# nickirk/pymes

Hardware: AMD Instinct MI355X
Metric: ccsd_iteration_time (lower is better)
Workload: dtype f64

## Files before the change

### pymes_amd/csrc/kernels.hip

```cpp
#include <hip/hip_runtime.h>
#include <type_traits>

#include <algorithm>
#include <atomic>
#include <chrono>
#include <cmath>
#include <cstdio>
#include <cstdlib>
#include <cstring>
#include <mutex>
#include <stdexcept>
#include <string>
#include <vector>

#include "../../include/pymes_amd.h"
#include "device_api.h"
#include "diis_small.h"
#include "device_util.h"
#include "launch.h"

namespace {

constexpr int kThreads = 256;
constexpr int BK = 16;

struct GemmK {
    const double* A;
    const double* B;
    double* C;
    const double* Cin;
    long a_ld, b_ld, ldc;
    int M, N, K;
    int Mc, Nc;
    double alpha, beta;
    int tiles_m, tiles_n;
    int nsplit, kchunk;
    long tile_begin;
    long nb2;
    long a_b1, a_b2, b_b1, b_b2, c_b1, c_b2;
    double* ws;
    long whole = 0, tail = 0;
    int mixed = 0;
    int fat = 0;
};
__host__ __device__ inline long glds_fat_slot(int fat) { return (long)((fat & 1) ? 144 : 128) * ((fat & 2) ? 144 : 128); }

__device__ __forceinline__ long xcd_remap(long b, long nblk) {
    const long q = nblk >> 3, r = nblk & 7;
    const long xcd = b & 7, pos = b >> 3;
    return (xcd < r ? xcd * (q + 1) : r * (q + 1) + (xcd - r) * q) + pos;
}

__device__ __forceinline__ void gemm_tile_rc(const GemmK& g, const long gt, int& tm, int& tn) {
    const int tiles = g.tiles_m * g.tiles_n;
    const int t = (int)(gt - (gt / tiles) * tiles);
    int rows = g.tiles_m, cols = g.tiles_n;
    if (g.fat) {
        rows -= g.fat & 1;
        cols -= (g.fat >> 1) & 1;
        int e = t - rows * cols;
        if (e >= 0) {
            if (g.fat & 1) {
                if (e < cols) { tm = rows; tn = e; return; }
                e -= cols;
            }
            tm = e;
            tn = cols;
            return;
        }
    }
    const int group_sz = 8 * cols;
    const int grp = t / group_sz;
    const int gm = min(rows - grp * 8, 8);
    const int tin = t - grp * group_sz;
    tm = grp * 8 + tin % gm;
    tn = tin / gm;
}

template <int BM, int BN, bool AKC, bool BKC, int VEC, bool STREAM = false>
__device__ __forceinline__ void dgemm_body(const GemmK& g, const long bid) {
    extern __shared__ __attribute__((aligned(16))) double smem[];
    constexpr int WM = BM / 2, WN = BN / 2;
    constexpr int FM = WM / 16, FN = WN / 16;
    constexpr int A_PITCH = AKC ? (BK + 2) : (BM + 16);
    constexpr int A_ROWS = AKC ? BM : BK;
    constexpr int A_TILE = A_PITCH * A_ROWS;
    constexpr int B_PITCH = BKC ? (BK + 2) : (BN + 16);
    constexpr int B_ROWS = BKC ? BN : BK;
    constexpr int B_TILE = B_PITCH * B_ROWS;
    constexpr int LA = BM * BK / (kThreads * VEC);
    constexpr int LB = BN * BK / (kThreads * VEC);
    constexpr int A_CH = (AKC ? BK : BM) / VEC;
    constexpr int B_CH = (BKC ? BK : BN) / VEC;
    constexpr int A_RSTEP = kThreads / A_CH;
    constexpr int B_RSTEP = kThreads / B_CH;

    double* As = smem;
    double* Bs = smem + (STREAM ? 1 : 2) * A_TILE;

    const int tid = threadIdx.x;
    const int lane = tid & 63, wave = tid >> 6;
    const int wm = wave >> 1, wn = wave & 1;
    const int l15 = lane & 15, l4 = lane >> 4;

    const int tiles = g.tiles_m * g.tiles_n;
    const long lt = bid / g.nsplit;
    const int ks = (int)(bid - lt * g.nsplit);
    const long gt = g.tile_begin + lt;
    const long z = gt / tiles;
    const int t = (int)(gt - z * tiles);
    constexpr int GROUP = 8;
    const int group_sz = GROUP * g.tiles_n;
    const int grp = t / group_sz;
    const int first_m = grp * GROUP;
    const int gm = min(g.tiles_m - first_m, GROUP);
    const int tin = t - grp * group_sz;
    const int tm = first_m + tin % gm;
    const int tn = tin / gm;
    const long z1 = z / g.nb2, z2 = z - z1 * g.nb2;

    const double* __restrict__ A = g.A + z1 * g.a_b1 + z2 * g.a_b2;
    const double* __restrict__ B = g.B + z1 * g.b_b1 + z2 * g.b_b2;
    const int m0 = tm * BM, n0 = tn * BN;
    const int kbeg = ks * g.kchunk;
    const int kend = min(g.K, kbeg + g.kchunk);
    const int nkt = (kend - kbeg + BK - 1) / BK;

    const int a_r = tid / A_CH, a_c = (tid % A_CH) * VEC;
    const int b_r = tid / B_CH, b_c = (tid % B_CH) * VEC;
    const double* pa[LA];
    const double* pb[LB];
#pragma unroll
    for (int i = 0; i < LA; ++i) {
        const int r = a_r + i * A_RSTEP;
        if (AKC) pa[i] = A + (long)min(m0 + r, g.M - 1) * g.a_ld + (kbeg + a_c);
        else pa[i] = A + (long)(kbeg + r) * g.a_ld + min(m0 + a_c, g.Mc - VEC);
    }
#pragma unroll
    for (int i = 0; i < LB; ++i) {
        const int r = b_r + i * B_RSTEP;
        if (BKC) pb[i] = B + (long)min(n0 + r, g.N - 1) * g.b_ld + (kbeg + b_c);
        else pb[i] = B + (long)(kbeg + r) * g.b_ld + min(n0 + b_c, g.Nc - VEC);
    }
    const long a_step = AKC ? (long)BK : (long)BK * g.a_ld;
    const long b_step = BKC ? (long)BK : (long)BK * g.b_ld;

    double ra[LA * VEC], rb[LB * VEC];

    auto load_full = [&]() {
#pragma unroll
        for (int i = 0; i < LA; ++i) {
            if constexpr (VEC == 2) {
                const v2d v = *reinterpret_cast<const v2d*>(pa[i]);
                ra[2 * i] = v[0];
// ... 1770 lines not shown
        if (c < nv && d < nv && c >= d) {
            const double x1 = sA[y][tx], x2 = sB[tx][y];
            Vp[row * npp + (long)c * (c + 1) / 2 + d] = x1 + x2;
            if (c > d) Vm[row * npm + (long)c * (c - 1) / 2 + d] = (a > b) ? x1 - x2 : 0.0;
        }
    }
}

constexpr int kFacK = 16;
__global__ void __launch_bounds__(256) ladder_pack_V_factors_kernel(const double* __restrict__ B, double* __restrict__ Vp,
                                                                    double* __restrict__ Vm, int naux, int n, int no, long rp0,
                                                                    long ntp, long npp, long npm) {
    __shared__ double sAc[kFacK][33], sBc[kFacK][33], sAd[kFacK][33], sBd[kFacK][33];
    const long bid = blockIdx.x;
    const long row = bid / ntp;
    const long tp = bid - row * ntp;
    int a, b, tc, td;
    unrank_pair(rp0 + row, a, b);
    unrank_pair(tp, tc, td);
    const int nv = n - no, c0 = tc * 32, d0 = td * 32;
    const long nn = (long)n * n;
    const double* __restrict__ Ba = B + (long)(no + a) * n + no;
    const double* __restrict__ Bb = B + (long)(no + b) * n + no;
    const int t = threadIdx.x, lane = t & 63, w = t >> 6;
    const int wc = (w >> 1) * 16, wd = (w & 1) * 16, l15 = lane & 15, l4 = lane >> 4;
    const int lx = t & 31, lk = t >> 5;
    v4d X = {0.0, 0.0, 0.0, 0.0}, Y = {0.0, 0.0, 0.0, 0.0};
    for (int q0 = 0; q0 < naux; q0 += kFacK) {
#pragma unroll
        for (int h = 0; h < 2; ++h) {
            const int k = lk + 8 * h, q = q0 + k;
            const long qo = (long)q * nn;
            const bool cok = q < naux && c0 + lx < nv, dok = q < naux && d0 + lx < nv;
            sAc[k][lx] = cok ? Ba[qo + c0 + lx] : 0.0;
            sBc[k][lx] = cok ? Bb[qo + c0 + lx] : 0.0;
            sAd[k][lx] = dok ? Ba[qo + d0 + lx] : 0.0;
            sBd[k][lx] = dok ? Bb[qo + d0 + lx] : 0.0;
        }
        __syncthreads();
#pragma unroll
        for (int kk = 0; kk < kFacK; kk += 4) {
            const int k = kk + l4;
            X = __builtin_amdgcn_mfma_f64_16x16x4f64(sAc[k][wc + l15], sBd[k][wd + l15], X, 0, 0, 0);
            Y = __builtin_amdgcn_mfma_f64_16x16x4f64(sBc[k][wc + l15], sAd[k][wd + l15], Y, 0, 0, 0);
        }
        __syncthreads();
    }
    const int d = d0 + wd + l15;
#pragma unroll
    for (int i = 0; i < 4; ++i) {
        const int c = c0 + wc + l4 + 4 * i;
        if (c < nv && d < nv && c >= d) {
            Vp[row * npp + (long)c * (c + 1) / 2 + d] = X[i] + Y[i];
            if (c > d) Vm[row * npm + (long)c * (c - 1) / 2 + d] = (a > b) ? X[i] - Y[i] : 0.0;
        }
    }
}

constexpr int kDirT = 64, kDirK = 8, kDirP = 80;
__global__ void __launch_bounds__(256, 4) direct_rows_fused_kernel(const double* __restrict__ Bvv, double* __restrict__ Vp,
                                                                double* __restrict__ Vm, int nv, int xp, long apitch, int nstage,
                                                                long rp0, long ntp, long npp, long npm) {
    __shared__ __attribute__((aligned(16))) double sm[2][4][kDirK][kDirP];
    const long bid = blockIdx.x;
    const long row = bid / ntp;
    const long tp = bid - row * ntp;
    int a, b, tc, td;
    unrank_pair(rp0 + row, a, b);
    unrank_pair(tp, tc, td);
    const int c0 = tc * kDirT, d0 = td * kDirT;
    const int t = threadIdx.x, lane = t & 63, w = t >> 6;
    const int wc = (w >> 1) * 32, wd = (w & 1) * 32, l15 = lane & 15, l4 = lane >> 4;
    const bool work = c0 + wc < nv && d0 + wd < nv && c0 + wc + 31 >= d0 + wd;
    const int sk = t >> 5, sx = (t & 31) * 2;
    const double* __restrict__ gA = Bvv + a * apitch + (long)sk * xp + sx;
    const double* __restrict__ gB = Bvv + b * apitch + (long)sk * xp + sx;
    const long step = (long)kDirK * xp;
    v2d r0, r1, r2, r3;
    auto fetch = [&](long o) {
        r0 = *reinterpret_cast<const v2d*>(gA + o + c0);
        r1 = *reinterpret_cast<const v2d*>(gB + o + d0);
        r2 = *reinterpret_cast<const v2d*>(gB + o + c0);
        r3 = *reinterpret_cast<const v2d*>(gA + o + d0);
    };
    auto stash = [&](int buf) {
        *reinterpret_cast<v2d*>(&sm[buf][0][sk][sx]) = r0;
        *reinterpret_cast<v2d*>(&sm[buf][1][sk][sx]) = r1;
        *reinterpret_cast<v2d*>(&sm[buf][2][sk][sx]) = r2;
        *reinterpret_cast<v2d*>(&sm[buf][3][sk][sx]) = r3;
    };
    fetch(0);
    stash(0);
    __syncthreads();
    v4d X[2][2], Y[2][2];
#pragma unroll
    for (int i = 0; i < 2; ++i)
#pragma unroll
        for (int j = 0; j < 2; ++j) X[i][j] = Y[i][j] = v4d{0.0, 0.0, 0.0, 0.0};
    for (int st = 0; st < nstage; ++st) {
        const int buf = st & 1;
        const bool more = st + 1 < nstage;
        if (more) fetch((long)(st + 1) * step);
        if (work) {
#pragma unroll
            for (int kk = 0; kk < kDirK; kk += 4) {
                const int k = kk + l4;
                double xa[2], xb[2], ya[2], yb[2];
#pragma unroll
                for (int i = 0; i < 2; ++i) {
                    xa[i] = sm[buf][0][k][wc + 16 * i + l15];
                    xb[i] = sm[buf][1][k][wd + 16 * i + l15];
                    ya[i] = sm[buf][2][k][wc + 16 * i + l15];
                    yb[i] = sm[buf][3][k][wd + 16 * i + l15];
                }
#pragma unroll
                for (int i = 0; i < 2; ++i)
#pragma unroll
                    for (int j = 0; j < 2; ++j) {
                        X[i][j] = __builtin_amdgcn_mfma_f64_16x16x4f64(xa[i], xb[j], X[i][j], 0, 0, 0);
                        Y[i][j] = __builtin_amdgcn_mfma_f64_16x16x4f64(ya[i], yb[j], Y[i][j], 0, 0, 0);
                    }
            }
        }
        if (more) stash(buf ^ 1);
        __syncthreads();
    }
    if (!work) return;
    double* __restrict__ vp = Vp + row * npp;
    double* __restrict__ vm = Vm + row * npm;
#pragma unroll
    for (int i = 0; i < 2; ++i)
#pragma unroll
        for (int j = 0; j < 2; ++j) {
            const int d = d0 + wd + 16 * j + l15;
#pragma unroll
            for (int e = 0; e < 4; ++e) {
                const int c = c0 + wc + 16 * i + l4 + 4 * e;
                if (c < nv && d < nv && c >= d) {
                    vp[(long)c * (c + 1) / 2 + d] = X[i][j][e] + Y[i][j][e];
                    if (c > d) vm[(long)c * (c - 1) / 2 + d] = (a > b) ? X[i][j][e] - Y[i][j][e] : 0.0;
                }
            }
        }
}

__global__ void ladder_dress_tfrag_kernel(const double* __restrict__ t1, double* __restrict__ tf, int no, int nv, int nk, long total) {
    const long e = blockIdx.x * (long)blockDim.x + threadIdx.x;
    if (e >= total) return;
    const int L = (int)(e & 63), kk = (int)((e >> 6) % nk), tile = (int)((e >> 6) / nk);
    const int a = 16 * tile + (L & 15), k = 4 * kk + (L >> 4);
    tf[e] = (a < nv && k < no) ? -t1[(long)a * no + k] : 0.0;
}

template <int NK>
__global__ void __launch_bounds__(64) ladder_dress_kernel(const double* __restrict__ V, const double* __restrict__ Pk,
                                                          const double* __restrict__ tf, double* __restrict__ W, int no,
                                                          int nv, long ld, long row0, long row1, double sgn, long ntp) {
    constexpr int TP = 16 * 16 + 16;
    __shared__ double turn[16 * TP];
    const int lane = threadIdx.x, g = lane >> 4, c = lane & 15;
    const long idx = blockIdx.x >> 3;
    const long cdb = (blockIdx.x & 7) + 8 * (idx / ntp), tp = idx % ntp;
    if (cdb * 16 >= ld) return;
    int ta_, tb_;
    unrank_pair(tp, ta_, tb_);
    const int a0 = ta_ * 16, b0 = tb_ * 16;
    const long tri0 = (long)a0 * (a0 + 1) / 2;
    if (tri0 + (long)15 * a0 + 120 + b0 + 15 < row0 || tri0 + b0 >= row1) return;
    double ta[NK], tb[NK];
#pragma unroll
    for (int kk = 0; kk < NK; ++kk) {
        ta[kk] = tf[((long)ta_ * NK + kk) * 64 + lane];
        tb[kk] = tf[((long)tb_ * NK + kk) * 64 + lane];
    }
    typedef unsigned v2u __attribute__((ext_vector_type(2)));
    constexpr unsigned kOff = 0x80000000u;
    const long col = cdb * 16 + c;
    const unsigned lo = (unsigned)(8 * ((long)g * ld + col));
    const unsigned lo_last = (unsigned)(8 * ((long)(min(4 * (NK - 1) + g, no - 1) - 4 * (NK - 1)) * ld + col));
    const unsigned ldb = (unsigned)(8 * ld);
    const __amdgpu_buffer_rsrc_t rPa = __builtin_amdgcn_make_buffer_rsrc(const_cast<double*>(Pk + (long)a0 * no * ld), 0, kOff, 0x00020000);
    const __amdgpu_buffer_rsrc_t rPb = __builtin_amdgcn_make_buffer_rsrc(const_cast<double*>(Pk + (long)b0 * no * ld), 0, kOff, 0x00020000);
    const __amdgpu_buffer_rsrc_t rV = __builtin_amdgcn_make_buffer_rsrc(const_cast<double*>(V + (tri0 - row0) * ld), 0, kOff, 0x00020000);
    const __amdgpu_buffer_rsrc_t rW = __builtin_amdgcn_make_buffer_rsrc(W + (tri0 - row0) * ld, 0, kOff, 0x00020000);
    unsigned vo[4];
#pragma unroll
    for (int r = 0; r < 4; ++r) {
        const long a = a0 + g + 4 * r;
        vo[r] = a < nv ? (unsigned)(8 * ((a * (a + 1) / 2 - tri0) * ld + col)) : kOff;
    }
    auto row_off = [&](int r, int x) {
        const int a = a0 + g + 4 * r;
        const long row = (long)a * (a + 1) / 2 + x;
        return (x <= a && row >= row0 && row < row1) ? vo[r] : kOff;
    };
    constexpr int PA = 1, NBP = 2 * (PA + 1), VA = 3, NBV = 2 * (VA + 1);
    double pf[NBP][NK], vin[NBV][4];
    auto fetch_p = [&](int n) {
        const int x0 = n < 16 ? a0 : b0, i = n < 16 ? n : n - 16;
        const unsigned so = (unsigned)(min(x0 + i, nv - 1) - x0) * (unsigned)no * ldb;
        const __amdgpu_buffer_rsrc_t rs = n < 16 ? rPa : rPb;
#pragma unroll
        for (int kk = 0; kk < NK - 1; ++kk)
            pf[n % NBP][kk] = __builtin_bit_cast(double, __builtin_amdgcn_raw_buffer_load_b64(rs, lo, so + 4u * kk * ldb, 0));
        pf[n % NBP][NK - 1] = __builtin_bit_cast(double, __builtin_amdgcn_raw_buffer_load_b64(rs, lo_last, so + 4u * (NK - 1) * ldb, 0));
    };
    auto fetch_v = [&](int n) {
        const int x = b0 + n - 16;
#pragma unroll
        for (int r = 0; r < 4; ++r)
            vin[n % NBV][r] = __builtin_bit_cast(double, __builtin_amdgcn_raw_buffer_load_b64(rV, row_off(r, x), (unsigned)x * ldb, 2));
    };
#pragma unroll
    for (int n = 0; n < 2 * PA; ++n) fetch_p(n);
#pragma unroll
    for (int p = 0; p < 8; ++p) {
        const int n0 = 2 * p, n1 = n0 + 1;
        fetch_p(n0 + 2 * PA);
        fetch_p(n1 + 2 * PA);
        if (n0 + 2 * VA >= 16) { fetch_v(n0 + 2 * VA); fetch_v(n1 + 2 * VA); }
        v4d acc0 = {0.0, 0.0, 0.0, 0.0}, acc1 = {0.0, 0.0, 0.0, 0.0};
#pragma unroll
        for (int kk = 0; kk < NK; ++kk) {
            acc0 = __builtin_amdgcn_mfma_f64_16x16x4f64(tb[kk], pf[n0 % NBP][kk], acc0, 0, 0, 0);
            acc1 = __builtin_amdgcn_mfma_f64_16x16x4f64(tb[kk], pf[n1 % NBP][kk], acc1, 0, 0, 0);
        }
#pragma unroll
        for (int rb = 0; rb < 4; ++rb) {
            turn[n0 * TP + (g + 4 * rb) * 16 + c] = acc0[rb];
            turn[n1 * TP + (g + 4 * rb) * 16 + c] = acc1[rb];
        }
    }
    __builtin_amdgcn_fence(__ATOMIC_SEQ_CST, "wavefront");
    __builtin_amdgcn_wave_barrier();
    const double s2 = sgn > 0.0 ? -1.0 : 1.0;
#pragma unroll
    for (int p = 0; p < 8; ++p) {
        const int b = 2 * p, n0 = 16 + b, n1 = n0 + 1;
        if (n0 + 2 * PA < 32) { fetch_p(n0 + 2 * PA); fetch_p(n1 + 2 * PA); }
        if (n0 + 2 * VA < 32) { fetch_v(n0 + 2 * VA); fetch_v(n1 + 2 * VA); }
        v4d acc0, acc1;
#pragma unroll
        for (int r = 0; r < 4; ++r) {
            acc0[r] = fma(s2, turn[(g + 4 * r) * TP + b * 16 + c], vin[n0 % NBV][r]);
            acc1[r] = fma(s2, turn[(g + 4 * r) * TP + (b + 1) * 16 + c], vin[n1 % NBV][r]);
        }
#pragma unroll
        for (int kk = 0; kk < NK; ++kk) {
            acc0 = __builtin_amdgcn_mfma_f64_16x16x4f64(ta[kk], pf[n0 % NBP][kk], acc0, 0, 0, 0);
            acc1 = __builtin_amdgcn_mfma_f64_16x16x4f64(ta[kk], pf[n1 % NBP][kk], acc1, 0, 0, 0);
        }
#pragma unroll
        for (int h = 0; h < 2; ++h) {
            const int bb = b0 + b + h;
#pragma unroll
            for (int r = 0; r < 4; ++r) {
                const double val = (sgn > 0.0 && a0 + g + 4 * r == bb) ? 0.0 : (double)(h ? acc1[r] : acc0[r]);
                __builtin_amdgcn_raw_buffer_store_b64(__builtin_bit_cast(v2u, val), rW, row_off(r, bb), (unsigned)bb * ldb, 2);
            }
        }
    }
}

struct PackTK {
    const double* T; const double* t1; double* Sp; double* Am;
    long ldp, ldm, rp0;
    int no, nv, flags;
};
__device__ __forceinline__ void ladder_pack_T_body(const PackTK& k, const unsigned vb) {
    const double* __restrict__ T = k.T;
    const double* __restrict__ t1 = k.t1;
    double* __restrict__ Sp = k.Sp;
    double* __restrict__ Am = k.Am;
    const int no = k.no, nv = k.nv, flags = k.flags;
    const long ldp = k.ldp, ldm = k.ldm;
    const long row = k.rp0 + vb;
    int c, d;
    unrank_pair(row, c, d);
    const bool row_half = flags & dev::PACK_ROW_HALF, prow = flags & dev::PACK_AM_PROWS,
               col_half = flags & dev::PACK_COL_HALF, pcol = flags & dev::PACK_AM_PCOLS;
    const long o2 = (long)no * no;
    const double* __restrict__ T1 = T ? T + ((long)c * nv + d) * o2 : nullptr;
    const double* __restrict__ T2 = T ? T + ((long)d * nv + c) * o2 : nullptr;
    const double fr = (c == d && row_half) ? 0.25 : 0.5;
    const long mrow = prow ? row : (long)c * (c - 1) / 2 + d;
    const bool has_m = prow || c > d;
    if (threadIdx.x == 0) {
        const long opp = (long)no * (no + 1) / 2, mcols = pcol ? opp : opp - no;
        if (ldp > opp) Sp[row * ldp + opp] = 0.0;
        if (has_m && ldm > mcols) Am[mrow * ldm + mcols] = 0.0;
    }
    for (int e = threadIdx.x; e < o2; e += blockDim.x) {
        const int i = e / no, j = e - i * no;
        if (i < j) continue;
        double x1 = 0.0, x2 = 0.0;
        if (T) { x1 = T1[e]; x2 = T2[e]; }
        if (t1) {
            x1 += t1[(long)c * no + i] * t1[(long)d * no + j];
            x2 += t1[(long)d * no + i] * t1[(long)c * no + j];
        }
        Sp[row * ldp + (long)i * (i + 1) / 2 + j] = ((i == j && col_half) ? 0.5 * fr : fr) * (x1 + x2);
        if (has_m && (pcol || i > j)) {
            const long mcol = pcol ? (long)i * (i + 1) / 2 + j : (long)i * (i - 1) / 2 + j;
            Am[mrow * ldm + mcol] = (c > d && i > j) ? 0.5 * (x1 - x2) : 0.0;
        }
    }
}
__global__ void ladder_pack_T_kernel(const PackTK k) { ladder_pack_T_body(k, blockIdx.x); }

struct UnpackK {
    const double* L; double* R;
    double beta;
    long total;
    int no, nv;
};
__device__ __forceinline__ void ladder_unpack_body(const UnpackK& k, const unsigned vb, const unsigned vgrid) {
    const double* __restrict__ L = k.L;
    double* __restrict__ R = k.R;
    const double beta = k.beta;
    const int no = k.no, nv = k.nv;
    const long total = k.total;
    const long opp = (long)no * (no + 1) / 2, ld = (long)no * no;
    for (long idx = vb * (long)blockDim.x + threadIdx.x; idx < total; idx += (long)vgrid * blockDim.x) {
        long r = idx;
        const int j = (int)(r % no); r /= no;
        const int i = (int)(r % no); r /= no;
        const int b = (int)(r % nv);
        const int a = (int)(r / nv);
        const int ah = max(a, b), al = min(a, b), ih = max(i, j), il = min(i, j);
        const double* __restrict__ row = L + ((long)ah * (ah + 1) / 2 + al) * ld;
        double v = row[(long)ih * (ih + 1) / 2 + il];
        if (a != b && i != j) {
            const double x = row[opp + (long)ih * (ih - 1) / 2 + il];
            v += ((a > b) == (i > j)) ? x : -x;
        }
        R[idx] = (beta != 0.0) ? beta * R[idx] + v : v;
    }
}
__global__ void ladder_unpack_kernel(const UnpackK k) { ladder_unpack_body(k, blockIdx.x, gridDim.x); }

struct RingOpK {
    const double* Wd; const double* Ud; double* M; double* N1;
    double a1, a2;
    int no, nv;
};
__device__ __forceinline__ void ring_operands_body(const RingOpK& q, const unsigned vb) {
    const double* __restrict__ Wd = q.Wd;
    const double* __restrict__ Ud = q.Ud;
    double* __restrict__ M = q.M;
    double* __restrict__ N1 = q.N1;
    const double a1 = q.a1, a2 = q.a2;
    const int no = q.no, nv = q.nv;
    extern __shared__ double tile[];
    constexpr int CT = 32;
    const int k = vb / nv, b = vb - k * nv;
    const long ov = (long)no * nv;
    const double* __restrict__ wd = Wd + ((long)k * nv + b) * ((long)nv * no);
    const double* __restrict__ ud = Ud + ((long)k * nv + b) * ((long)no * nv);
    const long col = (long)b * no;
    for (int c0 = 0; c0 < nv; c0 += CT) {
        const int nc = min(CT, nv - c0);
        for (int e = threadIdx.x; e < no * CT; e += blockDim.x) {
            const int j = e / CT, cc = e - j * CT;
            if (cc < nc) tile[j * (CT + 1) + cc] = ud[(long)j * nv + c0 + cc];
        }
        __syncthreads();
        for (int e = threadIdx.x; e < nc * no; e += blockDim.x) {
            const int cc = e / no, j = e - cc * no;
            const double u = tile[j * (CT + 1) + cc];
            const double w = wd[(long)(c0 + cc) * no + j];
            const long off = ((long)(c0 + cc) * no + k) * ov + col + j;
            N1[off] = -u;
            M[off] = a1 * w - a2 * u;
        }
        __syncthreads();
    }
}
__global__ void __launch_bounds__(256) ring_operands_kernel(const RingOpK q) { ring_operands_body(q, blockIdx.x); }

struct LayoutsK {
    const double* T; double* Td; double* Tx; double* Ttd;
    double ca, cb;
    int no, nv;
};
template <bool RESIDUAL>
__device__ __forceinline__ void t2_layouts_body(const LayoutsK& k, const unsigned vb) {
    const double* __restrict__ T = k.T;
    double* __restrict__ Td = k.Td;
    double* __restrict__ Tx = k.Tx;
    double* __restrict__ Ttd = k.Ttd;
    const int no = k.no, nv = k.nv;
    const double ca = k.ca, cb = k.cb;
    extern __shared__ double tile[];
    const int a = vb / nv, b = vb - a * nv;
    const long o2 = (long)no * no, ov = (long)no * nv;
    const double* __restrict__ Tab = T + ((long)a * nv + b) * o2;
    const double* __restrict__ Tba = T + ((long)b * nv + a) * o2;
    const long base = (long)a * no * ov + (long)b * no;
    for (int e = threadIdx.x; e < o2; e += blockDim.x) {
        const int i = e / no, j = e - i * no;
        const double x = Tab[e];
        tile[i * (no + 1) + j] = x;
        const long off = base + (long)i * ov + j;
        if (Td) Td[off] = x;
        Ttd[off] = RESIDUAL ? 2.0 * x - Tba[e] : ca * x + cb * Tba[e];
    }
    __syncthreads();
    for (int e = threadIdx.x; e < o2; e += blockDim.x) {
        const int j = e / no, i = e - j * no;
        Tx[base + (long)j * ov + i] = tile[i * (no + 1) + j];
    }
}
// ... 2450 lines not shown
            for (int i = 0; i < done[t].mm; ++i)
                for (int j = 0; j < done[t].nn; ++j) {
                    const double v = g_gram_host[dv][64 * t + i * done[t].NN + j];
                    const int gi = done[t].i0 + i, gj = done[t].j0 + j;
                    if (swap) out_host[(long)gj * n + gi] = v;
                    else out_host[(long)gi * n + gj] = v;
                }
        done.clear();
    };
    for (int i0 = 0; i0 < mx; i0 += 16)
        for (int j0 = 0; j0 < ny; j0 += 4) {
            const int mm = std::min(16, mx - i0), nn = std::min(4, ny - j0);
            int NN = 4;
            double* tile = tiles + 64 * done.size();
            if (mm <= 4) gram_tile_n<4>(X + i0, mm, Y + j0, nn, (long)len, vec, nblk, ws, tile, st, NN);
            else if (mm <= 8) gram_tile_n<8>(X + i0, mm, Y + j0, nn, (long)len, vec, nblk, ws, tile, st, NN);
            else if (mm <= 12) gram_tile_n<12>(X + i0, mm, Y + j0, nn, (long)len, vec, nblk, ws, tile, st, NN);
            else gram_tile_n<16>(X + i0, mm, Y + j0, nn, (long)len, vec, nblk, ws, tile, st, NN);
            done.push_back({i0, mm, j0, nn, NN});
            if ((int)done.size() == kGramTiles) flush();
        }
    flush();
}

void lincomb_multi(int m, int n, const double* const* x, const double* c, const double* beta, double* const* y, int64_t len,
                   stream_t s) {
    if (n <= 0 || len <= 0) return;
    if (m < 0 || m > 64 || n > 64) throw std::runtime_error("lincomb_multi: at most 64 inputs and 64 outputs per call");
    if (m > 16 || n > 4)
        for (int j = 0; j < n; ++j)
            for (int i = 0; i < m; ++i)
                if (y[j] == x[i]) throw std::runtime_error("lincomb_multi: an output may alias an input only for m <= 16, n <= 4");
    hipStream_t st = (hipStream_t)s;
    bool vec = true;
    for (int i = 0; i < m; ++i) vec = vec && aligned16(x[i]);
    for (int j = 0; j < n; ++j) vec = vec && aligned16(y[j]);
    double one[4] = {1.0, 1.0, 1.0, 1.0}, b0[4];
    for (int j0 = 0; j0 < n; j0 += 4) {
        const int nn = std::min(4, n - j0);
        for (int j = 0; j < nn; ++j) b0[j] = beta ? beta[j0 + j] : 0.0;
        if (m == 0) {
            const double* none[1] = {y[j0]};
            const double zero[4] = {0.0, 0.0, 0.0, 0.0};
            lincomb_multi_tile_n<4>(none, 1, zero, 4, b0, y + j0, nn, (long)len, vec, st);
            continue;
        }
        for (int i0 = 0; i0 < m; i0 += 16) {
            const int mm = std::min(16, m - i0);
            const double* bb = i0 == 0 ? b0 : one;
            const double* cc = c + (long)i0 * n + j0;
            if (mm <= 4) lincomb_multi_tile_n<4>(x + i0, mm, cc, n, bb, y + j0, nn, (long)len, vec, st);
            else if (mm <= 8) lincomb_multi_tile_n<8>(x + i0, mm, cc, n, bb, y + j0, nn, (long)len, vec, st);
            else if (mm <= 12) lincomb_multi_tile_n<12>(x + i0, mm, cc, n, bb, y + j0, nn, (long)len, vec, st);
            else lincomb_multi_tile_n<16>(x + i0, mm, cc, n, bb, y + j0, nn, (long)len, vec, st);
        }
    }
}

void cmul(const double* mr, const double* mi, const double* xr, const double* xi, double* yr, double* yi, int64_t n, stream_t s) {
    if (n <= 0) return;
    launch_kernel(cmul_kernel, dim3(grid_for(n)), dim3(256), 0, (hipStream_t)s, mr, mi, xr, xi, yr, yi, (long)n);
}

void exchange_split(const double* u, double* us, double* w, double* dg, int no, int nv, stream_t s) {
    const long total = (long)nv * nv * no * no;
    if (!total) return;
    launch_kernel(exchange_split_kernel, dim3(grid_for(total, 256, 256 * 64)), dim3(256), 0, (hipStream_t)s, u, us, w, dg, no, nv,
                       total);
}
void sgn_ij_add(double* D, const double* R, int no, int nv, stream_t s) {
    const long total = (long)nv * nv * no * no;
    if (!total) return;
    launch_kernel(sgn_ij_add_kernel, dim3(grid_for(total, 256, 256 * 64)), dim3(256), 0, (hipStream_t)s, D, R, no, total);
}
int64_t eom_diag_ws_doubles(int no, int nv) { return EomDiagWs(no, nv).total; }
void eom_diagonals(const double* V, const double* T, const double* dai, const double* iaai, const double* iaia, const double* ijij,
                   const double* abab, double* d1, double* d2, int no, int nv, double* ws, stream_t s) {
    hipStream_t st = (hipStream_t)s;
    const EomDiagWs w(no, nv);
    const long total = (long)nv * nv * no * no;
    if (w.total > 0x7fffffffL) throw std::runtime_error("eom_diagonals: problem too large for one grid");
    launch_kernel(eom_diag_sums_kernel, dim3((unsigned)w.total), dim3(256), 0, st, V, T, ws, no, nv);
    launch_kernel(eom_diag_singles_kernel, dim3((unsigned)(((long)nv * no + 255) / 256)), dim3(256), 0, st, ws, dai, iaai, iaia,
                       d1, no, nv);
    launch_kernel(eom_diag_doubles_kernel, dim3(grid_for(total, 256, 256 * 64)), dim3(256), 0, st, V, T, ws, dai, iaai, iaia, ijij,
                       abab, d2, no, nv, total);
}
void cshift_inv(const double* d, double zr, double zi, double hr, double hi, double shift, double* mr, double* mi, int64_t n,
                stream_t s) {
    if (n <= 0) return;
    launch_kernel(cshift_inv_kernel, dim3(grid_for(n)), dim3(256), 0, (hipStream_t)s, d, zr, zi, hr, hi, shift, mr, mi, (long)n);
}

void tau_build(double* tau, const double* t2, const double* t1, int no, int nv, stream_t s) {
    const long total = (long)nv * nv * no * no;
    if (!total) return;
    const TauK k{tau, t2, t1, total, no, nv};
    const double cost = 16.0 * (double)total / 4.0e6;
    if (phase_open((hipStream_t)s) && phase_small(cost)) {
        PhaseRec& t = phase_push(PK_TAU, 0, grid_for(total), 0, cost, k);
        phase_reads(t, {prange(t2, total), prange(t1, (long)no * nv)});
        phase_writes(t, {prange(tau, total)});
        return;
    }
    launch_kernel(tau_kernel, dim3(grid_for(total)), dim3(256), 0, (hipStream_t)s, k);
}

void ladder_pack_V(const double* V, double* Vp, double* Vm, int nr, int nc, int64_t rp0, int64_t rp1, stream_t s, int64_t ldvp,
                   int64_t ldvm) {
    if (rp1 <= rp0) return;
    const long npp = ldvp ? (long)ldvp : (long)nc * (nc + 1) / 2, npm = ldvm ? (long)ldvm : (long)nc * (nc - 1) / 2;
    const int nt = (nc + 31) / 32;
    const long ntp = (long)nt * (nt + 1) / 2;
    const long nblk = (rp1 - rp0) * ntp;
    if (nblk > 0x7fffffffL) throw std::runtime_error("ladder_pack_V: grid too large");
    launch_kernel(ladder_pack_V_kernel, dim3((unsigned)nblk), dim3(256), 0, (hipStream_t)s, V, Vp, Vm, nr, nc,
                       (long)rp0, nt, ntp, npp, npm);
}

void ladder_pack_V_factors(const double* B, double* Vp, double* Vm, int naux, int n, int no, int64_t rp0, int64_t rp1,
                           stream_t s, int64_t ldvp, int64_t ldvm) {
    if (rp1 <= rp0) return;
    const int nv = n - no;
    if (naux < 1 || no < 0 || nv < 1 || rp0 < 0 || rp1 > (int64_t)nv * (nv + 1) / 2)
        throw std::runtime_error("ladder_pack_V_factors: bad shape or pair-row range");
    const long npp = ldvp ? (long)ldvp : (long)nv * (nv + 1) / 2, npm = ldvm ? (long)ldvm : (long)nv * (nv - 1) / 2;
    const int nt = (nv + 31) / 32;
    const long ntp = (long)nt * (nt + 1) / 2;
    const long nblk = (rp1 - rp0) * ntp;
    if (nblk > 0x7fffffffL) throw std::runtime_error("ladder_pack_V_factors: grid too large");
    launch_kernel(ladder_pack_V_factors_kernel, dim3((unsigned)nblk), dim3(256), 0, (hipStream_t)s, B, Vp, Vm, naux, n, no,
                 (long)rp0, ntp, npp, npm);
}

bool direct_rows_fused_ok() { return true; }

void direct_rows_fused(const double* Bvv, double* Vp, double* Vm, int nv, int64_t qp, int64_t xp, int64_t rp0, int64_t rp1,
                       stream_t s, int64_t ldvp, int64_t ldvm) {
    if (rp1 <= rp0) return;
    const long npair = (long)nv * (nv + 1) / 2;
    if (nv < 1 || qp < kDirK || qp % kDirK || xp < nv || xp % kDirT || rp0 < 0 || rp1 > npair || ldvp < npair ||
        ldvm < std::max<long>(npair - nv, 1) || xp > 0x7fffffffL || qp / kDirK > 0x7fffffffL)
        throw std::runtime_error("direct_rows_fused: bad shape, padding or pair-row range");
    const int nt = (nv + kDirT - 1) / kDirT;
    const long ntp = (long)nt * (nt + 1) / 2;
    const long nblk = (rp1 - rp0) * ntp;
    if (nblk > 0x7fffffffL) throw std::runtime_error("direct_rows_fused: grid too large");
    launch_kernel(direct_rows_fused_kernel, dim3((unsigned)nblk), dim3(256), 0, (hipStream_t)s, Bvv, Vp, Vm, nv, (int)xp,
                  (long)(qp * xp), (int)(qp / kDirK), (long)rp0, ntp, (long)ldvp, (long)ldvm);
}

bool ladder_dress_ok(int no, int nv) {
    const double ld = (double)((((long)nv * (nv + 1) / 2) + 15) & ~15L);
    return no >= 1 && no <= PYMES_NOCC_MAX_BRA_DRESS && nv >= 1 && 8.0 * ld * (15.0 * nv + 137.0) < 2147483648.0;
}

int64_t ladder_dress_ws_doubles(int no, int nv) { return (int64_t)((nv + 15) / 16) * ((no + 3) / 4) * 64; }

void ladder_dress(const double* V, const double* Pk, const double* t1, double* W, int no, int nv, int64_t ld, int64_t row0,
                  int64_t row1, double sgn, double* ws, stream_t s) {
    if (!ladder_dress_ok(no, nv)) throw std::runtime_error("ladder_dress: nocc outside 1.." + std::to_string(PYMES_NOCC_MAX_BRA_DRESS) + " or tile extents beyond 2 GB");
    if (ld <= 0 || (ld & 15)) throw std::runtime_error("ladder_dress: the row pitch must be a multiple of 16 doubles");
    if ((reinterpret_cast<uintptr_t>(V) | reinterpret_cast<uintptr_t>(Pk) | reinterpret_cast<uintptr_t>(W)) & 127)
        throw std::runtime_error("ladder_dress: operands must be 128-byte aligned");
    if (!ws) throw std::runtime_error("ladder_dress: workspace missing");
    const long npp = (long)nv * (nv + 1) / 2;
    if (row0 < 0 || row1 > npp || row0 > row1) throw std::runtime_error("ladder_dress: bad pair-row range");
    if (row1 == row0) return;
    const long nt = (nv + 15) / 16, ntp = nt * (nt + 1) / 2, ncdb = ld / 16, nblk = 8 * ((ncdb + 7) / 8) * ntp;
    if (nblk > 0x7fffffffL) throw std::runtime_error("ladder_dress: grid too large");
    if (8.0 * (double)ld * (15.0 * nv + 137.0) >= 2147483648.0) throw std::runtime_error("ladder_dress: tile extent exceeds the 2-GB buffer window");
    const dim3 grid((unsigned)nblk), block(64);
    hipStream_t st = (hipStream_t)s;
    const int nk = (no + 3) / 4;
    const long nfrag = ladder_dress_ws_doubles(no, nv);
    launch_kernel(ladder_dress_tfrag_kernel, dim3((unsigned)((nfrag + 255) / 256)), dim3(256), 0, st, t1, ws, no, nv, nk, nfrag);
#define PYMES_DRESS(NK) case NK: launch_kernel(ladder_dress_kernel<NK>, grid, block, 0, st, V, Pk, (const double*)ws, W, no, nv, (long)ld, (long)row0, (long)row1, sgn, ntp); break;
    switch (nk) {
        PYMES_DRESS(1) PYMES_DRESS(2) PYMES_DRESS(3) PYMES_DRESS(4) PYMES_DRESS(5) PYMES_DRESS(6) PYMES_DRESS(7) PYMES_DRESS(8)
        PYMES_DRESS(9) PYMES_DRESS(10) PYMES_DRESS(11) PYMES_DRESS(12) PYMES_DRESS(13) PYMES_DRESS(14) PYMES_DRESS(15) PYMES_DRESS(16)
        PYMES_DRESS(17) PYMES_DRESS(18) PYMES_DRESS(19) PYMES_DRESS(20)
    }
#undef PYMES_DRESS
}

void ladder_pack_T(const double* X, const double* t1, double* Sp, double* Am, int nc, int nr, int flags, int64_t ldp,
                   int64_t ldm, stream_t s, int64_t rp0, int64_t rp1) {
    const long npp = (long)nr * (nr + 1) / 2, opp = (long)nc * (nc + 1) / 2, opm = (long)nc * (nc - 1) / 2;
    if (!ldp) ldp = opp;
    if (!ldm) ldm = (flags & PACK_AM_PCOLS) ? opp : opm;
    if (!X && !t1) throw std::runtime_error("ladder_pack_T: nothing to pack");
    if (rp1 < 0) { rp0 = 0; rp1 = npp; }
    if (rp0 < 0 || rp1 > npp || rp0 > rp1) throw std::runtime_error("ladder_pack_T: bad row range");
    if ((rp0 != 0 || rp1 != npp) && !(flags & PACK_AM_PROWS)) throw std::runtime_error("ladder_pack_T: a row range needs PACK_AM_PROWS");
    if (rp1 == rp0) return;
    const PackTK k{X, t1, Sp, Am, (long)ldp, (long)ldm, (long)rp0, nc, nr, flags};
    const double cost = 24.0 * (double)(rp1 - rp0) * (double)nc * (double)nc / 4.0e6;
    if (phase_open((hipStream_t)s) && phase_small(cost)) {
        PhaseRec& t = phase_push(PK_PACK_T, 0, rp1 - rp0, 0, cost, k);
        phase_reads(t, {prange(X, X ? (long)nr * nr * nc * nc : 0), prange(t1, t1 ? (long)nr * nc : 0)});
        const long am_rows = (flags & PACK_AM_PROWS) ? npp : (long)nr * (nr - 1) / 2;
        phase_writes(t, {pbox(Sp + rp0 * ldp, {{rp1 - rp0, ldp}, {ldp, 1}}),
                         (flags & PACK_AM_PROWS) ? pbox(Am + rp0 * ldm, {{rp1 - rp0, ldm}, {ldm, 1}}) : prange(Am, am_rows * ldm)});
        return;
    }
    launch_kernel(ladder_pack_T_kernel, dim3((unsigned)(rp1 - rp0)), dim3(256), 0, (hipStream_t)s, k);
}

void ladder_unpack(const double* L, double* R, double beta, int no, int nv, stream_t s) {
    const long total = (long)nv * nv * no * no;
    if (!total) return;
    const UnpackK k{L, R, beta, total, no, nv};
    const double cost = 20.0 * (double)total / 4.0e6;
    if (phase_open((hipStream_t)s) && phase_small(cost)) {
        PhaseRec& t = phase_push(PK_LADDER_UNPACK, 0, grid_for(total), 0, cost, k);
        phase_reads(t, {prange(L, (long)nv * (nv + 1) / 2 * no * no)});
        phase_writes(t, {prange(R, total)});
        return;
    }
    launch_kernel(ladder_unpack_kernel, dim3(grid_for(total)), dim3(256), 0, (hipStream_t)s, k);
}

constexpr size_t kPairTileBudget = 64 * 1024;
constexpr size_t pair_tile_bytes(size_t no) { return no * (no + 1) * sizeof(double); }
static_assert(pair_tile_bytes(PYMES_NOCC_MAX_FUSED) <= kPairTileBudget && pair_tile_bytes(PYMES_NOCC_MAX_FUSED + 1) > kPairTileBudget,
              "PYMES_NOCC_MAX_FUSED is the largest nocc whose tile fits the budget");
bool fused_pair_kernels_ok(int no) { return no <= PYMES_NOCC_MAX_FUSED; }

void ring_operands(const double* Viabj, const double* Viajb, double* M, double* N1, double a1, double a2, int no, int nv,
                   stream_t s) {
    if (no < 1 || nv < 1) return;
    const size_t lds = sizeof(double) * (size_t)no * 33;
    if (lds > 64 * 1024) throw std::runtime_error("ring_operands: nocc too large for the LDS tile");
    const RingOpK k{Viabj, Viajb, M, N1, a1, a2, no, nv};
    const long ov2 = (long)no * nv * no * nv;
    const double cost = 32.0 * (double)ov2 / 4.0e6;
    if (phase_open((hipStream_t)s) && phase_small(cost)) {
        PhaseRec& t = phase_push(PK_RING_OPERANDS, 0, (long)no * nv, (int)lds, cost, k);
        phase_reads(t, {prange(Viabj, ov2), prange(Viajb, ov2)});
        phase_writes(t, {prange(M, ov2), prange(N1, ov2)});
        return;
    }
    launch_kernel(ring_operands_kernel, dim3((unsigned)((long)no * nv)), dim3(256), lds, (hipStream_t)s, k);
}

void t2_layouts(const double* T, double* Td, double* Tx, double* Ttd, int no, int nv, stream_t s, double ca, double cb) {
    if (!fused_pair_kernels_ok(no)) throw std::runtime_error("t2_layouts: nocc too large for the LDS tile");
    const size_t lds = sizeof(double) * no * (no + 1);
    const LayoutsK k{T, Td, Tx, Ttd, ca, cb, no, nv};
    const bool res = ca == 2.0 && cb == -1.0;
    const long n4 = (long)nv * nv * no * no;
    const double cost = 40.0 * (double)n4 / 4.0e6;
    if (phase_open((hipStream_t)s) && phase_small(cost)) {
        PhaseRec& t = phase_push(PK_T2_LAYOUTS, res ? 1 : 0, (long)nv * nv, (int)lds, cost, k);
        phase_reads(t, {prange(T, n4)});
        phase_writes(t, {prange(Td, Td ? n4 : 0), prange(Tx, n4), prange(Ttd, n4)});
        return;
    }
    if (res) launch_kernel(t2_layouts_kernel<true>, dim3((unsigned)(nv * nv)), dim3(256), lds, (hipStream_t)s, k);
    else launch_kernel(t2_layouts_kernel<false>, dim3((unsigned)(nv * nv)), dim3(256), lds, (hipStream_t)s, k);
}
void t2_layouts_sym(const double* T, double* Td, double* Tx, double* Ttd, int no, int nv, stream_t s) {
    if (!fused_pair_kernels_ok(no)) throw std::runtime_error("t2_layouts: nocc too large for the LDS tile");
    const long n4 = (long)nv * nv * no * no;
    phase_open((hipStream_t)s);
    if (phase_small(40.0 * (double)n4 / 4.0e6)) {
        t2_layouts(T, Td, Tx, Ttd, no, nv, s);
        return;
    }
    if (!n4) return;
    const LayoutsK k{T, Td, Tx, Ttd, 2.0, -1.0, no, nv};
    launch_kernel(t2_layouts_sym_kernel, dim3((unsigned)(nv * nv)), dim3(256), sizeof(double) * no * (no + 1), (hipStream_t)s, k);
}

void residual_assemble(const double* V, const double* L, const double* N, const double* D, const double* X, double* R,
                       int no, int nv, stream_t s, double xd) {
    if (!fused_pair_kernels_ok(no)) throw std::runtime_error("residual_assemble: nocc too large for the LDS tile");
    const size_t lds = sizeof(double) * no * (no + 1);
    const AssembleK k{V, L, N, D, X, R, xd, no, nv};
    const long n4 = (long)nv * nv * no * no;
    const double cost = 48.0 * (double)n4 / 4.0e6;
    if (phase_open((hipStream_t)s) && phase_small(cost)) {
        PhaseRec& t = phase_push(PK_ASSEMBLE, 0, (long)nv * (nv + 1) / 2, (int)lds, cost, k);
        phase_reads(t, {prange(V, V ? n4 : 0), prange(L, L ? (long)nv * (nv + 1) / 2 * no * no : 0), prange(N, n4), prange(D, n4), prange(X, n4)});
        phase_writes(t, {prange(R, n4)});
        return;
    }
    launch_kernel(residual_assemble_kernel, dim3((unsigned)((long)nv * (nv + 1) / 2)), dim3(256), lds, (hipStream_t)s, k);
}

void pairs_pack(const double* full, double* Xc, int no, int nv, int64_t r0, int64_t r1, stream_t s) {
    if (r1 <= r0) return;
    launch_kernel(pairs_pack_kernel, dim3((unsigned)(r1 - r0)), dim3(256), 0, (hipStream_t)s, full, Xc, no, nv, (long)r0);
}
void energy_norms_pairs(const double* f, const double* t1, const double* tc, const double* Edir, const double* Eex,
                        const double* dtc, int no, int nv, int64_t r0, int64_t r1, bool with_t1, double out_host[6],
                        stream_t s) {
    hipStream_t st = (hipStream_t)s;
    const int dv = current_device();
    ensure_dot_ws(dv);
    const long npairs = std::max<long>(0, (long)(r1 - r0));
    const int nb = (int)std::max<long>(1, std::min<long>(kDotBlocks, 2 * npairs));
    launch_kernel(energy_norms_pairs_kernel, dim3(nb), dim3(256), 0, st, f, t1, tc, Edir, Eex, dtc, no, nv, (long)r0,
                       npairs, with_t1 ? 1 : 0, g_dot_ws[dv]);
    double* out_dev = g_dot_ws[dv] + 16 * kDotBlocks;
    launch_kernel(dots_stage2_kernel, dim3(6), dim3(256), 0, st, g_dot_ws[dv], nb, out_dev);
    HIP_CHECK(copy_async(g_dot_host[dv], out_dev, sizeof(double) * 6, hipMemcpyDeviceToHost, st));
    wait_idle(st);
    for (int i = 0; i < 6; ++i) out_host[i] = g_dot_host[dv][i];
}
void energy_norms_pairs_dev(const double* f, const double* t1, const double* tc, const double* Edir, const double* Eex,
                            const double* dtc, int no, int nv, int64_t r0, int64_t r1, bool with_t1, double* out_dev,
                            stream_t s) {
    hipStream_t st = (hipStream_t)s;
    const int dv = current_device();
    ensure_dot_ws(dv);
    const long npairs = std::max<long>(0, (long)(r1 - r0));
    const int nb = (int)std::max<long>(1, std::min<long>(kDotBlocks, 2 * npairs));
    launch_kernel(energy_norms_pairs_kernel, dim3(nb), dim3(256), 0, st, f, t1, tc, Edir, Eex, dtc, no, nv, (long)r0,
                       npairs, with_t1 ? 1 : 0, g_dot_ws[dv]);
    launch_kernel(dots_stage2_kernel, dim3(6), dim3(256), 0, st, g_dot_ws[dv], nb, out_dev);
}
void pairs_unpack(const double* Xc, double* full, int no, int nv, int64_t r0, int64_t r1, stream_t s) {
    if (r1 <= r0) return;
// ... 205 lines not shown
```

Before: 0.1572.

## Restructure ladder dress kernel with global-to-LDS DMA pipeline and fused accumulation

Rewrites the ladder dress kernel so the Pk panels stream through a four-slot LDS ring using direct global-to-LDS loads, with explicit vmcnt waits. Both the tb and ta contractions now accumulate into one set of 16 MFMA accumulators instead of staging an intermediate through shared memory. V is loaded up front as 128-bit vectors, and the output goes through a swizzled LDS transpose before 128-bit stores. The aim is to hide load latency and cut LDS round-trips and narrow memory ops, at the cost of many more live registers and hand-tuned waitcnt logic. A new guard rejects shapes whose panel offsets would overflow 32-bit lane offsets.

```diff
diff --git a/pymes_amd/csrc/kernels.hip b/pymes_amd/csrc/kernels.hip
--- a/pymes_amd/csrc/kernels.hip
+++ b/pymes_amd/csrc/kernels.hip
@@ -1,5 +1,6 @@
 #include <hip/hip_runtime.h>
 #include <type_traits>
+#include <utility>
 
 #include <algorithm>
 #include <atomic>
@@ -2076,112 +2077,143 @@
     tf[e] = (a < nv && k < no) ? -t1[(long)a * no + k] : 0.0;
 }
 
+template <class F, int... I>
+__device__ __forceinline__ void dress_units(F&& f, std::integer_sequence<int, I...>) { (f(std::integral_constant<int, I>{}), ...); }
+template <int N>
+__device__ __forceinline__ void dress_wait_vm() { asm volatile("s_waitcnt vmcnt(%0) lgkmcnt(0)" ::"n"(N) : "memory"); }
+
 template <int NK>
 __global__ void __launch_bounds__(64) ladder_dress_kernel(const double* __restrict__ V, const double* __restrict__ Pk,
                                                           const double* __restrict__ tf, double* __restrict__ W, int no,
                                                           int nv, long ld, long row0, long row1, double sgn, long ntp) {
-    constexpr int TP = 16 * 16 + 16;
-    __shared__ double turn[16 * TP];
-    const int lane = threadIdx.x, g = lane >> 4, c = lane & 15;
+    constexpr int U = 2 * NK;
+    __shared__ __attribute__((aligned(16))) double sm[4 * 1024];
+    const int lane = threadIdx.x;
     const long idx = blockIdx.x >> 3;
     const long cdb = (blockIdx.x & 7) + 8 * (idx / ntp), tp = idx % ntp;
     if (cdb * 16 >= ld) return;
     int ta_, tb_;
     unrank_pair(tp, ta_, tb_);
+    ta_ = uni(ta_);
+    tb_ = uni(tb_);
     const int a0 = ta_ * 16, b0 = tb_ * 16;
     const long tri0 = (long)a0 * (a0 + 1) / 2;
     if (tri0 + (long)15 * a0 + 120 + b0 + 15 < row0 || tri0 + b0 >= row1) return;
+    const double s2 = sgn > 0.0 ? -1.0 : 1.0;
     double ta[NK], tb[NK];
 #pragma unroll
     for (int kk = 0; kk < NK; ++kk) {
         ta[kk] = tf[((long)ta_ * NK + kk) * 64 + lane];
-        tb[kk] = tf[((long)tb_ * NK + kk) * 64 + lane];
-    }
-    typedef unsigned v2u __attribute__((ext_vector_type(2)));
+        tb[kk] = s2 * tf[((long)tb_ * NK + kk) * 64 + lane];
+    }
+#pragma unroll
+    for (int kk = 0; kk < NK; ++kk) asm volatile("" : "+v"(ta[kk]), "+v"(tb[kk]));
+    const unsigned ldb = (unsigned)(8 * ld);
+    const char* pbase[2] = {uni_ptr(Pk + (long)a0 * no * ld + cdb * 16), uni_ptr(Pk + (long)b0 * no * ld + cdb * 16)};
+    unsigned po[2][2];
+#pragma unroll
+    for (int s = 0; s < 2; ++s)
+#pragma unroll
+        for (int h = 0; h < 2; ++h) {
+            const int x0 = s ? b0 : a0;
+            const unsigned x = (unsigned)(min(x0 + 8 * h + (lane >> 3), nv - 1) - x0);
+            po[s][h] = x * (unsigned)no * ldb + 16u * (unsigned)((lane & 7) ^ (4 * h + (lane >> 4)));
+        }
+    const unsigned lds0 = uni((int)lds_addr_of(sm));
+    auto dma = [&](int u, int i) {
+        const int kr = min(4 * (u >> 1) + (i >> 1), no - 1);
+        glds16_su(pbase[u & 1] + (long)kr * ldb, po[u & 1][i & 1], lds0 + (unsigned)((u & 3) * 8192 + i * 1024));
+    };
+    v2d fr[2][8];
+    const int fsw = (lane >> 1) & 7;
+    auto reads = [&](int u) {
+#pragma unroll
+        for (int m = 0; m < 8; ++m) fr[u & 1][m] = *reinterpret_cast<const v2d*>(sm + (u & 3) * 1024 + lane * 16 + 2 * (m ^ fsw));
+    };
+    typedef unsigned v4u __attribute__((ext_vector_type(4)));
     constexpr unsigned kOff = 0x80000000u;
-    const long col = cdb * 16 + c;
-    const unsigned lo = (unsigned)(8 * ((long)g * ld + col));
-    const unsigned lo_last = (unsigned)(8 * ((long)(min(4 * (NK - 1) + g, no - 1) - 4 * (NK - 1)) * ld + col));
-    const unsigned ldb = (unsigned)(8 * ld);
-    const __amdgpu_buffer_rsrc_t rPa = __builtin_amdgcn_make_buffer_rsrc(const_cast<double*>(Pk + (long)a0 * no * ld), 0, kOff, 0x00020000);
-    const __amdgpu_buffer_rsrc_t rPb = __builtin_amdgcn_make_buffer_rsrc(const_cast<double*>(Pk + (long)b0 * no * ld), 0, kOff, 0x00020000);
     const __amdgpu_buffer_rsrc_t rV = __builtin_amdgcn_make_buffer_rsrc(const_cast<double*>(V + (tri0 - row0) * ld), 0, kOff, 0x00020000);
     const __amdgpu_buffer_rsrc_t rW = __builtin_amdgcn_make_buffer_rsrc(W + (tri0 - row0) * ld, 0, kOff, 0x00020000);
-    unsigned vo[4];
-#pragma unroll
-    for (int r = 0; r < 4; ++r) {
-        const long a = a0 + g + 4 * r;
-        vo[r] = a < nv ? (unsigned)(8 * ((a * (a + 1) / 2 - tri0) * ld + col)) : kOff;
-    }
-    auto row_off = [&](int r, int x) {
-        const int a = a0 + g + 4 * r;
-        const long row = (long)a * (a + 1) / 2 + x;
-        return (x <= a && row >= row0 && row < row1) ? vo[r] : kOff;
+    const int bl = lane >> 3;
+    const unsigned vo[2] = {(unsigned)(8 * ((long)bl * ld + cdb * 16 + 2 * (lane & 7))),
+                            (unsigned)(8 * ((long)(bl + 8) * ld + cdb * 16 + 2 * (lane & 7)))};
+    auto row_so = [&](int j) {
+        const long a = a0 + (j >> 1);
+        return (unsigned)(a * (a + 1) / 2 - tri0 + b0) * ldb;
     };
-    constexpr int PA = 1, NBP = 2 * (PA + 1), VA = 3, NBV = 2 * (VA + 1);
-    double pf[NBP][NK], vin[NBV][4];
-    auto fetch_p = [&](int n) {
-        const int x0 = n < 16 ? a0 : b0, i = n < 16 ? n : n - 16;
-        const unsigned so = (unsigned)(min(x0 + i, nv - 1) - x0) * (unsigned)no * ldb;
-        const __amdgpu_buffer_rsrc_t rs = n < 16 ? rPa : rPb;
-#pragma unroll
-        for (int kk = 0; kk < NK - 1; ++kk)
-            pf[n % NBP][kk] = __builtin_bit_cast(double, __builtin_amdgcn_raw_buffer_load_b64(rs, lo, so + 4u * kk * ldb, 0));
-        pf[n % NBP][NK - 1] = __builtin_bit_cast(double, __builtin_amdgcn_raw_buffer_load_b64(rs, lo_last, so + 4u * (NK - 1) * ldb, 0));
+    auto row_vo = [&](int j) {
+        const int a = a0 + (j >> 1), b = b0 + 8 * (j & 1) + bl;
+        const long row = (long)a * (a + 1) / 2 + b;
+        return (a < nv && b <= a && row >= row0 && row < row1) ? vo[j & 1] : kOff;
     };
-    auto fetch_v = [&](int n) {
-        const int x = b0 + n - 16;
-#pragma unroll
-        for (int r = 0; r < 4; ++r)
-            vin[n % NBV][r] = __builtin_bit_cast(double, __builtin_amdgcn_raw_buffer_load_b64(rV, row_off(r, x), (unsigned)x * ldb, 2));
+    v2d vin[32];
+    auto load_v = [&]() {
+#pragma unroll
+        for (int j = 0; j < 32; ++j)
+            vin[j] = __builtin_bit_cast(v2d, __builtin_amdgcn_raw_buffer_load_b128(rV, row_vo(j), row_so(j), 2));
     };
-#pragma unroll
-    for (int n = 0; n < 2 * PA; ++n) fetch_p(n);
-#pragma unroll
-    for (int p = 0; p < 8; ++p) {
-        const int n0 = 2 * p, n1 = n0 + 1;
-        fetch_p(n0 + 2 * PA);
-        fetch_p(n1 + 2 * PA);
-        if (n0 + 2 * VA >= 16) { fetch_v(n0 + 2 * VA); fetch_v(n1 + 2 * VA); }
-        v4d acc0 = {0.0, 0.0, 0.0, 0.0}, acc1 = {0.0, 0.0, 0.0, 0.0};
-#pragma unroll
-        for (int kk = 0; kk < NK; ++kk) {
-            acc0 = __builtin_amdgcn_mfma_f64_16x16x4f64(tb[kk], pf[n0 % NBP][kk], acc0, 0, 0, 0);
-            acc1 = __builtin_amdgcn_mfma_f64_16x16x4f64(tb[kk], pf[n1 % NBP][kk], acc1, 0, 0, 0);
-        }
-#pragma unroll
-        for (int rb = 0; rb < 4; ++rb) {
-            turn[n0 * TP + (g + 4 * rb) * 16 + c] = acc0[rb];
-            turn[n1 * TP + (g + 4 * rb) * 16 + c] = acc1[rb];
-        }
-    }
+    auto wait_landed = [&](int n) {
+        switch (n) {
+            case 0: dress_wait_vm<0>(); break;
+            case 8: dress_wait_vm<8>(); break;
+            case 16: dress_wait_vm<16>(); break;
+            case 32: dress_wait_vm<32>(); break;
+            case 40: dress_wait_vm<40>(); break;
+            default: dress_wait_vm<48>(); break;
+        }
+    };
+    v4d acc[16];
+#pragma unroll
+    for (int c = 0; c < 16; ++c) acc[c] = v4d{0.0, 0.0, 0.0, 0.0};
+#pragma unroll
+    for (int u = 0; u < 3 && u < U; ++u)
+#pragma unroll
+        for (int i = 0; i < 8; ++i) dma(u, i);
+    if (U < 4) load_v();
+    wait_landed(8 + (U > 2 ? 8 : 0) + (U < 4 ? 32 : 0));
+    reads(0);
+    auto unit = [&](auto uc) {
+        constexpr int u = decltype(uc)::value;
+        if constexpr (u + 1 < U) {
+            wait_landed((u + 2 < U ? 8 : 0) + ((U < 4 || u >= U - 3) ? 32 : 0));
+            reads(u + 1);
+        }
+        __builtin_amdgcn_sched_barrier(0);
+        constexpr int kk = u >> 1;
+#pragma unroll
+        for (int c = 0; c < 16; ++c) {
+            const double p = fr[u & 1][c >> 1][c & 1];
+            if constexpr ((u & 1) != 0) acc[c] = __builtin_amdgcn_mfma_f64_16x16x4f64(ta[kk], p, acc[c], 0, 0, 0);
+            else acc[c] = __builtin_amdgcn_mfma_f64_16x16x4f64(p, tb[kk], acc[c], 0, 0, 0);
+            if (c & 1) {
+                if constexpr (u + 3 < U) dma(u + 3, c >> 1);
+                __builtin_amdgcn_sched_barrier(0);
+            }
+        }
+        if constexpr (U >= 4 && u == U - 4) load_v();
+    };
+    dress_units(unit, std::make_integer_sequence<int, U>{});
+    const int osw = lane & 7;
+#pragma unroll
+    for (int r = 0; r < 4; ++r)
+#pragma unroll
+        for (int m = 0; m < 8; ++m)
+            *reinterpret_cast<v2d*>(sm + (64 * r + lane) * 16 + 2 * (m ^ osw)) = v2d{acc[2 * m][r], acc[2 * m + 1][r]};
     __builtin_amdgcn_fence(__ATOMIC_SEQ_CST, "wavefront");
     __builtin_amdgcn_wave_barrier();
-    const double s2 = sgn > 0.0 ? -1.0 : 1.0;
-#pragma unroll
-    for (int p = 0; p < 8; ++p) {
-        const int b = 2 * p, n0 = 16 + b, n1 = n0 + 1;
-        if (n0 + 2 * PA < 32) { fetch_p(n0 + 2 * PA); fetch_p(n1 + 2 * PA); }
-        if (n0 + 2 * VA < 32) { fetch_v(n0 + 2 * VA); fetch_v(n1 + 2 * VA); }
-        v4d acc0, acc1;
-#pragma unroll
-        for (int r = 0; r < 4; ++r) {
-            acc0[r] = fma(s2, turn[(g + 4 * r) * TP + b * 16 + c], vin[n0 % NBV][r]);
-            acc1[r] = fma(s2, turn[(g + 4 * r) * TP + (b + 1) * 16 + c], vin[n1 % NBV][r]);
-        }
-#pragma unroll
-        for (int kk = 0; kk < NK; ++kk) {
-            acc0 = __builtin_amdgcn_mfma_f64_16x16x4f64(ta[kk], pf[n0 % NBP][kk], acc0, 0, 0, 0);
-            acc1 = __builtin_amdgcn_mfma_f64_16x16x4f64(ta[kk], pf[n1 % NBP][kk], acc1, 0, 0, 0);
-        }
-#pragma unroll
-        for (int h = 0; h < 2; ++h) {
-            const int bb = b0 + b + h;
-#pragma unroll
-            for (int r = 0; r < 4; ++r) {
-                const double val = (sgn > 0.0 && a0 + g + 4 * r == bb) ? 0.0 : (double)(h ? acc1[r] : acc0[r]);
-                __builtin_amdgcn_raw_buffer_store_b64(__builtin_bit_cast(v2u, val), rW, row_off(r, bb), (unsigned)bb * ldb, 2);
-            }
+    const int ooff = bl * 16 + 2 * ((lane & 7) ^ bl);
+#pragma unroll
+    for (int j0 = 0; j0 < 32; j0 += 8) {
+        v2d o[8];
+#pragma unroll
+        for (int j = 0; j < 8; ++j) o[j] = *reinterpret_cast<const v2d*>(sm + (j0 + j) * 128 + ooff);
+        __builtin_amdgcn_sched_barrier(0);
+#pragma unroll
+        for (int j = 0; j < 8; ++j) {
+            const int jj = j0 + j;
+            v2d w = o[j] + vin[jj];
+            if (sgn > 0.0 && a0 + (jj >> 1) == b0 + 8 * (jj & 1) + bl) w = v2d{0.0, 0.0};
+            __builtin_amdgcn_raw_buffer_store_b128(__builtin_bit_cast(v4u, w), rW, row_vo(jj), row_so(jj), 2);
         }
     }
 }
@@ -4938,7 +4970,8 @@
 
 bool ladder_dress_ok(int no, int nv) {
     const double ld = (double)((((long)nv * (nv + 1) / 2) + 15) & ~15L);
-    return no >= 1 && no <= PYMES_NOCC_MAX_BRA_DRESS && nv >= 1 && 8.0 * ld * (15.0 * nv + 137.0) < 2147483648.0;
+    return no >= 1 && no <= PYMES_NOCC_MAX_BRA_DRESS && nv >= 1 && 8.0 * ld * (15.0 * nv + 137.0) < 2147483648.0 &&
+           120.0 * no * ld < 4294967296.0;
 }
 
 int64_t ladder_dress_ws_doubles(int no, int nv) { return (int64_t)((nv + 15) / 16) * ((no + 3) / 4) * 64; }
@@ -4956,6 +4989,7 @@
     const long nt = (nv + 15) / 16, ntp = nt * (nt + 1) / 2, ncdb = ld / 16, nblk = 8 * ((ncdb + 7) / 8) * ntp;
     if (nblk > 0x7fffffffL) throw std::runtime_error("ladder_dress: grid too large");
     if (8.0 * (double)ld * (15.0 * nv + 137.0) >= 2147483648.0) throw std::runtime_error("ladder_dress: tile extent exceeds the 2-GB buffer window");
+    if (120.0 * (double)no * (double)ld >= 4294967296.0) throw std::runtime_error("ladder_dress: panel extent exceeds the 4-GB lane offset");
     const dim3 grid((unsigned)nblk), block(64);
     hipStream_t st = (hipStream_t)s;
     const int nk = (no + 3) / 4;
```

Result: no change. 0.1566 (median of 6 runs) (-0.4%).
